# Ruyi-Zha/endosurf

Hardware: AMD Instinct MI355X
Metric: training rays/sec (1024 rays x 64 samples) (higher is better)
Workload: dtype f32

## Files before the change

endosurf_amd/csrc/chain_common.h:

```cpp
#pragma once
#include <hip/hip_runtime.h>

#include <type_traits>

#include "../../include/endosurf_hip.h"
#include "arch.h"

namespace es {

typedef float f32x16 __attribute__((ext_vector_type(16)));

__device__ __forceinline__ float relu1(float z) {
    float r;
    asm("v_max_f32_e32 %0, 0, %1" : "=v"(r) : "v"(z));
    return r;
}

constexpr int TM = 64;
constexpr int NTHREADS = 256;
constexpr int MAIN_FLOATS = HID * TM;
constexpr int AUX56_FLOATS = 56 * TM;
constexpr int LEAN_LDS_BYTES = (MAIN_FLOATS + AUX56_FLOATS + 256) * 4;

__device__ __forceinline__ int swz(int k, int r) { return k * TM + (r ^ ((k & 15) << 2)); }

template <int RTC, int NTC>
__device__ __forceinline__ void acc_zero(f32x16 (&acc)[RTC][NTC]) {
#pragma unroll
    for (int i = 0; i < RTC; ++i)
#pragma unroll
        for (int j = 0; j < NTC; ++j)
#pragma unroll
            for (int r = 0; r < 16; ++r) acc[i][j][r] = 0.f;
}

__device__ __forceinline__ float f4c(const float4& v, int j) { return j == 0 ? v.x : (j == 1 ? v.y : (j == 2 ? v.z : v.w)); }

template <int KG, int RTC, int NTC, int PF = 2>
__device__ __forceinline__ void gemm_seg(f32x16 (&acc)[RTC][NTC], const float* At, const float4* __restrict__ W,
                                         int rt0, int nt0, int lane) {
    static_assert(PF == 2 || PF == 4, "prefetch groups: even-group parity of the swizzle table");
    constexpr bool GUARD = (KG % (2 * PF)) != 0;
    const int lo = lane & 31, hi = lane >> 5;
    float4 b0[PF][NTC], b1[PF][NTC];
    const float4* wl = W + lane;
    int aoff[RTC][8];
#pragma unroll
    for (int ri = 0; ri < RTC; ++ri)
#pragma unroll
        for (int c = 0; c < 8; ++c) aoff[ri][c] = ((((rt0 + ri) * 32 + lo) ^ (hi << 2)) ^ (8 * c)) + 64 * hi;

    auto loadB = [&](float4(&b)[PF][NTC], int g0) {
#pragma unroll
        for (int gi = 0; gi < PF; ++gi)
#pragma unroll
            for (int ni = 0; ni < NTC; ++ni)
                if (!GUARD || g0 + gi < KG) b[gi][ni] = wl[(size_t)((nt0 + ni) * KG + g0 + gi) * 64];
    };
    auto comp = [&](const float4(&b)[PF][NTC], int g0) {
        const float* Ag = At + 512 * g0;
#pragma unroll
        for (int gi = 0; gi < PF; ++gi) {
            if (!GUARD || g0 + gi < KG) {
#pragma unroll
                for (int j = 0; j < 4; ++j) {
                    float a[RTC];
#pragma unroll
                    for (int ri = 0; ri < RTC; ++ri) a[ri] = Ag[aoff[ri][4 * (gi & 1) + j] + 512 * gi + 128 * j];
#pragma unroll
                    for (int ri = 0; ri < RTC; ++ri)
#pragma unroll
                        for (int ni = 0; ni < NTC; ++ni)
                            acc[ri][ni] = __builtin_amdgcn_mfma_f32_32x32x2f32(a[ri], f4c(b[gi][ni], j), acc[ri][ni], 0, 0, 0);
                }
            }
        }
    };

    loadB(b0, 0);
    if constexpr (KG > 2 * PF) {
#pragma unroll 1
        for (int g0 = 0; g0 < KG; g0 += 2 * PF) {
            if (!GUARD || g0 + PF < KG) loadB(b1, g0 + PF);
            comp(b0, g0);
            if (g0 + 2 * PF < KG) loadB(b0, g0 + 2 * PF);
            if (!GUARD || g0 + PF < KG) comp(b1, g0 + PF);
        }
    } else {
        if (PF < KG) loadB(b1, PF);
        comp(b0, 0);
        if (PF < KG) comp(b1, PF);
    }
}

template <int RTC, int NTC, class F>
__device__ __forceinline__ void for_quads(f32x16 (&acc)[RTC][NTC], int rt0, int nt0, int lane, F&& f) {
    const int lo = lane & 31, hi = lane >> 5;
#pragma unroll
    for (int ri = 0; ri < RTC; ++ri)
#pragma unroll
        for (int ni = 0; ni < NTC; ++ni)
#pragma unroll
            for (int q = 0; q < 4; ++q) {
                float v[4] = {acc[ri][ni][4 * q + 0], acc[ri][ni][4 * q + 1], acc[ri][ni][4 * q + 2], acc[ri][ni][4 * q + 3]};
                f((rt0 + ri) * 32 + 8 * q + 4 * hi, (nt0 + ni) * 32 + lo, v);
            }
}

template <int RTC, int NTC, class F>
__device__ __forceinline__ void for_quads_noacc(int rt0, int nt0, int lane, F&& f) {
    const int lo = lane & 31, hi = lane >> 5;
#pragma unroll
    for (int ri = 0; ri < RTC; ++ri)
#pragma unroll
        for (int ni = 0; ni < NTC; ++ni)
#pragma unroll
            for (int q = 0; q < 4; ++q) f((rt0 + ri) * 32 + 8 * q + 4 * hi, (nt0 + ni) * 32 + lo);
}

template <int RTC, int NTC, class F>
__device__ __forceinline__ void for_quads_qi(f32x16 (&acc)[RTC][NTC], int rt0, int nt0, int lane, F&& f) {
    const int lo = lane & 31, hi = lane >> 5;
#pragma unroll
    for (int ri = 0; ri < RTC; ++ri)
#pragma unroll
        for (int ni = 0; ni < NTC; ++ni)
#pragma unroll
            for (int q = 0; q < 4; ++q) {
                float v[4] = {acc[ri][ni][4 * q + 0], acc[ri][ni][4 * q + 1], acc[ri][ni][4 * q + 2], acc[ri][ni][4 * q + 3]};
                f((rt0 + ri) * 32 + 8 * q + 4 * hi, (nt0 + ni) * 32 + lo, v, (ri * NTC + ni) * 4 + q);
            }
}
template <int NI, class F>
__device__ __forceinline__ void for_quads_half(f32x16 (&acc)[2][2], int nt0, int lane, F&& f) {
    const int lo = lane & 31, hi = lane >> 5;
#pragma unroll
    for (int ri = 0; ri < 2; ++ri)
#pragma unroll
        for (int q = 0; q < 4; ++q) {
            float v[4] = {acc[ri][NI][4 * q + 0], acc[ri][NI][4 * q + 1], acc[ri][NI][4 * q + 2], acc[ri][NI][4 * q + 3]};
            f(ri * 32 + 8 * q + 4 * hi, (nt0 + NI) * 32 + lo, v, ri * 4 + q);
        }
}

typedef float f32x2v __attribute__((ext_vector_type(2)));
__device__ __forceinline__ void add_bias4(float (&v)[4], float b) {
    const f32x2v bb = {b, b};
    f32x2v lo = {v[0], v[1]}, hi = {v[2], v[3]};
    lo += bb; hi += bb;
    v[0] = lo[0]; v[1] = lo[1]; v[2] = hi[0]; v[3] = hi[1];
}
__device__ __forceinline__ float keep_if_bit(float v, unsigned w, int k) {
    const int m = __builtin_amdgcn_sbfe((int)w, k, 1);
    return __uint_as_float(__float_as_uint(v) & (unsigned)m);
}
template <int RTC> struct QuadOff { int o[RTC * 4]; };
template <int RTC>
__device__ __forceinline__ QuadOff<RTC> quad_offsets(int rt0, int nt0, int lane) {
    QuadOff<RTC> qo;
    const int lo = lane & 31, hi = lane >> 5;
#pragma unroll
    for (int ri = 0; ri < RTC; ++ri)
#pragma unroll
        for (int q = 0; q < 4; ++q) {
            int v = swz(nt0 * 32 + lo, (rt0 + ri) * 32 + 8 * q + 4 * hi);
            asm volatile("" : "+v"(v));
            qo.o[ri * 4 + q] = v;
        }
    return qo;
}
template <int RTC, int NTC, class F>
__device__ __forceinline__ void for_quads_off(f32x16 (&acc)[RTC][NTC], const QuadOff<RTC>& qo, int rt0, int nt0, int lane, F&& f) {
    const int lo = lane & 31, hi = lane >> 5;
#pragma unroll
    for (int ri = 0; ri < RTC; ++ri)
#pragma unroll
        for (int ni = 0; ni < NTC; ++ni)
#pragma unroll
            for (int q = 0; q < 4; ++q) {
                float v[4] = {acc[ri][ni][4 * q + 0], acc[ri][ni][4 * q + 1], acc[ri][ni][4 * q + 2], acc[ri][ni][4 * q + 3]};
                f((rt0 + ri) * 32 + 8 * q + 4 * hi, (nt0 + ni) * 32 + lo, v, qo.o[ri * 4 + q] + 2048 * ni, ni);
            }
}
__device__ __forceinline__ void lds_store_quad_at(float* At, int off, const float (&v)[4]) {
    *reinterpret_cast<float4*>(At + off) = make_float4(v[0], v[1], v[2], v[3]);
}
__device__ __forceinline__ void lds_store_quad(float* At, int col, int row, const float (&v)[4]) {
    *reinterpret_cast<float4*>(&At[swz(col, row)]) = make_float4(v[0], v[1], v[2], v[3]);
}
__device__ __forceinline__ void lds_load_quad(const float* At, int col, int row, float (&v)[4]) {
    const float4 t = *reinterpret_cast<const float4*>(&At[swz(col, row)]);
    v[0] = t.x; v[1] = t.y; v[2] = t.z; v[3] = t.w;
}
__device__ __forceinline__ void lds_add_quad(float* At, int col, int row, const float (&v)[4]) {
    float4* p = reinterpret_cast<float4*>(&At[swz(col, row)]);
    float4 t = *p;
    t.x += v[0]; t.y += v[1]; t.z += v[2]; t.w += v[3];
    *p = t;
}
__device__ __forceinline__ void g_store_quad(float* __restrict__ base, size_t grow0, int ld, int row, int col, const float (&v)[4]) {
    float* p = base + (grow0 + row) * (size_t)ld + col;
    __builtin_nontemporal_store(v[0], p); __builtin_nontemporal_store(v[1], p + ld);
    __builtin_nontemporal_store(v[2], p + 2 * ld); __builtin_nontemporal_store(v[3], p + 3 * ld);
}
__device__ __forceinline__ void g_load_quad(const float* __restrict__ base, size_t grow0, int ld, int row, int col, float (&v)[4]) {
    const float* p = base + (grow0 + row) * (size_t)ld + col;
    v[0] = __builtin_nontemporal_load(p); v[1] = __builtin_nontemporal_load(p + ld);
    v[2] = __builtin_nontemporal_load(p + 2 * ld); v[3] = __builtin_nontemporal_load(p + 3 * ld);
}

typedef float v4f_frag __attribute__((ext_vector_type(4)));
__device__ __forceinline__ size_t frag_off(size_t grow0, int row, int col) {
    const int ri = row >> 5, q = (row >> 3) & 3, hi = (row >> 2) & 1;
    const int w = col >> 6, ni = (col >> 5) & 1, lo = col & 31;
    return grow0 * 256 + (size_t)(((w * 16 + (ri * 2 + ni) * 4 + q) * 64 + hi * 32 + lo) * 4);
}
__device__ __forceinline__ void g_store_quad_f(float* __restrict__ base, size_t grow0, int row, int col, const float (&v)[4]) {
    const v4f_frag t = {v[0], v[1], v[2], v[3]};
    __builtin_nontemporal_store(t, reinterpret_cast<v4f_frag*>(base + frag_off(grow0, row, col)));
}
__device__ __forceinline__ void g_load_quad_f(const float* __restrict__ base, size_t grow0, int row, int col, float (&v)[4]) {
    const v4f_frag t = __builtin_nontemporal_load(reinterpret_cast<const v4f_frag*>(base + frag_off(grow0, row, col)));
    v[0] = t[0]; v[1] = t[1]; v[2] = t[2]; v[3] = t[3];
}
template <int RTC, int NTC>
__device__ __forceinline__ void prefetch_quads_f(float (&buf)[RTC * NTC * 4][4], const float* __restrict__ base, size_t grow0, int rt0, int nt0,
                                                 int lane) {
    const int lo = lane & 31, hi = lane >> 5;
#pragma unroll
    for (int ri = 0; ri < RTC; ++ri)
#pragma unroll
        for (int ni = 0; ni < NTC; ++ni)
#pragma unroll
            for (int q = 0; q < 4; ++q)
                g_load_quad_f(base, grow0, (rt0 + ri) * 32 + 8 * q + 4 * hi, (nt0 + ni) * 32 + lo, buf[(ri * NTC + ni) * 4 + q]);
}
template <int NI>
__device__ __forceinline__ void prefetch_half_f(float (&buf)[8][4], const float* __restrict__ base, size_t grow0, int nt0, int lane) {
    const int lo = lane & 31, hi = lane >> 5;
#pragma unroll
    for (int ri = 0; ri < 2; ++ri)
#pragma unroll
        for (int q = 0; q < 4; ++q) g_load_quad_f(base, grow0, ri * 32 + 8 * q + 4 * hi, (nt0 + NI) * 32 + lo, buf[ri * 4 + q]);
}

template <int NC>
__device__ __forceinline__ void load_tile(float* At, const float* __restrict__ src, size_t grow0, int ld, int tid) {
    const int r = tid >> 2, c4 = tid & 3;
    const float* p = src + (grow0 + r) * (size_t)ld;
#pragma unroll 4
    for (int jj = 0; jj < NC / 16; ++jj) {
        const int c = 4 * (c4 + 4 * jj);
        const float4 v = *reinterpret_cast<const float4*>(p + c);
        At[swz(c + 0, r)] = v.x; At[swz(c + 1, r)] = v.y; At[swz(c + 2, r)] = v.z; At[swz(c + 3, r)] = v.w;
    }
}
__device__ __forceinline__ void load_tile_256(float* At, const float* __restrict__ src, size_t grow0, int ld, int tid) {
    load_tile<256>(At, src, grow0, ld, tid);
}

struct MaskWords { unsigned w[2][2]; };
__device__ __forceinline__ MaskWords load_mask_words(const unsigned* __restrict__ Ml, int tile64, int wave, int lane) {
    MaskWords m;
    const unsigned* p = Ml + (size_t)(2 * tile64) * 256 + wave * 64 + (lane & 31);
    m.w[0][0] = p[0]; m.w[0][1] = p[32]; m.w[1][0] = p[256]; m.w[1][1] = p[256 + 32];
    return m;
}
__device__ __forceinline__ float mask_keep(float v, const MaskWords& m, int qi, int i, int hi) {
    const int ri_c = qi >> 3, ni = (qi >> 2) & 1, q_c = qi & 3;
    const int pq = ((q_c >> 1) * 2 + ni) * 4 + 2 * (q_c & 1) + hi;
    return keep_if_bit(v, m.w[ri_c][i >> 1], 2 * pq + (i & 1));
}
__device__ __forceinline__ bool mask_bit(const MaskWords& m, int qi, int i, int hi) {
    const int ri_c = qi >> 3, ni = (qi >> 2) & 1, q_c = qi & 3;
    const int pq = ((q_c >> 1) * 2 + ni) * 4 + 2 * (q_c & 1) + hi;
    return (m.w[ri_c][i >> 1] >> (2 * pq + (i & 1))) & 1u;
}

__device__ __forceinline__ float softplus100(float z) {
    const float e = __builtin_amdgcn_exp2f(-144.26950408889634f * fabsf(z));
    return fmaf(0.006931471805599453f, __builtin_amdgcn_logf(1.f + e), relu1(z));
}
__device__ __forceinline__ float softplus100_grad_from_s(float s) {
    const float x = 100.f * s;
    return x < 0.02f ? x * (1.f - x * (0.5f - x * (1.f / 6.f))) : 1.f - __expf(-x);
}

typedef float f32x2p __attribute__((ext_vector_type(2)));
__device__ __forceinline__ f32x2p softplus100_grad_from_s2(f32x2p s) {
    const f32x2p x = s * 100.f;
    const f32x2p t = x * -1.4426950408889634f;
    f32x2p e;
    e[0] = __builtin_amdgcn_exp2f(t[0]); e[1] = __builtin_amdgcn_exp2f(t[1]);
    const f32x2p big = 1.f - e;
    const f32x2p ser = x * (1.f - x * (0.5f - x * (1.f / 6.f)));
    f32x2p r;
    r[0] = x[0] < 0.02f ? ser[0] : big[0];
    r[1] = x[1] < 0.02f ? ser[1] : big[1];
    return r;
}
__device__ __forceinline__ void softplus100_grad_from_s4(const float (&s)[4], float (&d)[4]) {
    const f32x2p a = softplus100_grad_from_s2(f32x2p{s[0], s[1]}), b = softplus100_grad_from_s2(f32x2p{s[2], s[3]});
    d[0] = a[0]; d[1] = a[1]; d[2] = b[0]; d[3] = b[1];
}

__device__ __forceinline__ int enc_index(int D, int i, int fn, int c) { return D + (2 * i + fn) * D + c; }

template <int NOUT>
__device__ __forceinline__ void smalln_partial(const float* At, const float* __restrict__ Wrows, int ldw, float* scr, int tid) {
    const int row = tid & 63;
    const int part = __builtin_amdgcn_readfirstlane(tid >> 6);
    float s[NOUT];
#pragma unroll
    for (int i = 0; i < NOUT; ++i) s[i] = 0.f;
    const int k0 = part * 64;
#pragma unroll 8
    for (int kk = 0; kk < 64; ++kk) {
        const float a = At[swz(k0 + kk, row)];
#pragma unroll
        for (int i = 0; i < NOUT; ++i) s[i] = fmaf(Wrows[i * ldw + k0 + kk], a, s[i]);
    }
#pragma unroll
    for (int i = 0; i < NOUT; ++i) scr[(part * NOUT + i) * 64 + row] = s[i];
}
template <int NOUT>
__device__ __forceinline__ float smalln_reduce(const float* scr, int i, int row) {
    return (scr[(0 * NOUT + i) * 64 + row] + scr[(1 * NOUT + i) * 64 + row]) + (scr[(2 * NOUT + i) * 64 + row] + scr[(3 * NOUT + i) * 64 + row]);
}

struct PointSrc : ::es_points {};
static_assert(sizeof(PointSrc) == sizeof(es_points) && std::is_standard_layout<PointSrc>::value, "es::PointSrc is es_points");
__device__ __forceinline__ void load_point(const PointSrc& s, int i_in, float (&x)[3], float& t, float (&d)[3]) {
    int i = i_in;
    if (i >= s.M) { x[0] = x[1] = x[2] = 0.f; t = 0.f; d[0] = d[1] = 0.f; d[2] = 1.f; return; }
    if (s.mode == 0 || (s.mode == 2 && i >= s.M_split)) {
        if (s.mode == 2) i -= s.M_split;
        x[0] = s.x[3 * (size_t)i]; x[1] = s.x[3 * (size_t)i + 1]; x[2] = s.x[3 * (size_t)i + 2];
        t = s.t[s.t_scalar ? 0 : i];
        if (s.dirs) { d[0] = s.dirs[3 * (size_t)i]; d[1] = s.dirs[3 * (size_t)i + 1]; d[2] = s.dirs[3 * (size_t)i + 2]; }
        else { d[0] = d[1] = 0.f; d[2] = 1.f; }
    } else {
        const int ray = i / s.n_per_ray, smp = i - ray * s.n_per_ray;
        const float* r = s.rays + 9 * (size_t)ray;
        const float zz = s.z[(size_t)ray * s.ldz + smp];
        const float inv = r[5] + 1e-6f;
        d[0] = r[3]; d[1] = r[4]; d[2] = r[5];
        x[0] = r[0] + (r[3] / inv) * zz; x[1] = r[1] + (r[4] / inv) * zz; x[2] = r[2] + (r[5] / inv) * zz;
        t = r[8];
    }
}

}
```

endosurf_amd/csrc/point_bwd_bodies.h:

```cpp
#pragma once
#include <type_traits>

#include "chain_common.h"
#include "encode.h"
#include "tabs.h"
#include "workspace.h"

namespace es {

struct BwdArgs {
    PointSrc src;
    Tabs tb;
    const float4* packed;
    const float* weff;
    float* ws;
    WsLayout L;
    int flags;
    int M_color;
    const float* d_sdf;
    const float* d_go;
    const float* d_rgb;
};
__device__ __forceinline__ float* wsb(const BwdArgs& a, int buf) { return a.ws + a.L.off[buf]; }

// ... 271 lines not shown
        acc_zero(acc);
        const int seg = l <= 4 ? SF0 + l : SF0 + l + 1;
        gemm_seg<32, 2, 2>(acc, mainT, a.packed + a.tb.segoff[seg], 0, 2 * wave, lane);
        if (l == 4) gemm_seg<5, 2, 2>(acc, aux, a.packed + a.tb.segoff[SF4A], 0, 2 * wave, lane);
        __syncthreads();
        epi_t(acc, l);
        __syncthreads();
    }
    auto epi_b = [&](f32x16(&acc)[2][2], int l) {
        auto half = [&](auto NI) {
            float S[8][4], Z2[8][4];
            prefetch_half_f<decltype(NI)::value>(S, SACT + (size_t)(l - 1) * Mp * 256, grow0, 2 * wave, lane);
            prefetch_half_f<decltype(NI)::value>(Z2, ZB + (size_t)(l - 1) * Mp * 256, grow0, 2 * wave, lane);
            for_quads_half<decltype(NI)::value>(acc, 2 * wave, lane, [&](int row, int col, float(&v)[4], int b8) {
                float dphi[4];
                softplus100_grad_from_s4(S[b8], dphi);
#pragma unroll
                for (int h = 0; h < 2; ++h) {
                    const f32x2p d = {dphi[2 * h], dphi[2 * h + 1]}, t = {v[2 * h], v[2 * h + 1]}, z = {Z2[b8][2 * h], Z2[b8][2 * h + 1]};
                    const f32x2p o = d * t + z;
                    v[2 * h] = o[0]; v[2 * h + 1] = o[1];
                }
                lds_store_quad(mainT, col, row, v);
                g_store_quad_f(ZB + (size_t)(l - 1) * Mp * 256, grow0, row, col, v);
            });
        };
        half(std::integral_constant<int, 0>{});
        half(std::integral_constant<int, 1>{});
    };
    {
        f32x16 acc[2][2];
        acc_zero(acc);
        if (color) {
            load_tile_256(mainT, wsb(a, WS_FEATBAR), grow0, 256, tid);
            __syncthreads();
            gemm_seg<32, 2, 2>(acc, mainT, a.packed + a.tb.segoff[SR8F], 0, 2 * wave, lane);
            __syncthreads();
        }
        const float* w8 = a.weff + a.tb.woff[NET_S * LAYERS + 8];
        for_quads(acc, 0, 2 * wave, lane, [&](int row, int col, float(&v)[4]) {
            const float w = w8[col];
#pragma unroll
            for (int i = 0; i < 4; ++i) v[i] += sb[row + i] * w;
            float s[4], z2[4];
            g_load_quad_f(SACT + (size_t)7 * Mp * 256, grow0, row, col, s);
            g_load_quad_f(ZB + (size_t)7 * Mp * 256, grow0, row, col, z2);
#pragma unroll
            for (int i = 0; i < 4; ++i) v[i] = softplus100_grad_from_s(s[i]) * v[i] + z2[i];
            lds_store_quad(mainT, col, row, v);
            g_store_quad_f(ZB + (size_t)7 * Mp * 256, grow0, row, col, v);
        });
    }
    __syncthreads();
#pragma unroll 1
    for (int l = 7; l >= 1; --l) {
        f32x16 acc[2][2];
        acc_zero(acc);
        const int seg = l <= 4 ? SR0 + l : SR0 + l + 1;
        gemm_seg<32, 2, 2>(acc, mainT, a.packed + a.tb.segoff[seg], 0, 2 * wave, lane);
        f32x16 accA[1][1];
        if (l == 4) {
            acc_zero(accA);
            gemm_seg<32, 1, 1>(accA, mainT, a.packed + a.tb.segoff[SR4A], wave >> 1, wave & 1, lane);
        }
        __syncthreads();
        epi_b(acc, l);
        if (l == 4)
            for_quads(accA, wave >> 1, wave & 1, lane, [&](int row, int col, float(&v)[4]) { if (col < 40) lds_store_quad(aux, col, row, v); });
        __syncthreads();
    }
    {
        f32x16 accA[1][1];
        acc_zero(accA);
        gemm_seg<32, 1, 1>(accA, mainT, a.packed + a.tb.segoff[SR0], wave >> 1, wave & 1, lane);
        for_quads(accA, wave >> 1, wave & 1, lane, [&](int row, int col, float(&v)[4]) { if (col < 40) lds_add_quad(aux, col, row, v); });
    }
    __syncthreads();
    if (tid < 192) {
        const int j = tid >> 6, row = tid & 63;
        const float x = px[j * 64 + row];
        float g = enc3_adjoint<6>(aux, 0, j, row, x);
        const float* AE = wsb(a, WS_S_ADJEPS) + (grow0 + row) * 64;
        float h = 0.f;
#pragma unroll
        for (int i = 0; i < 6; ++i) {
            const float f = (float)(1 << i);
            float s, co;
            sincosf(x * f, &s, &co);
            h -= f * f * (AE[enc_index(3, i, 0, j)] * s + AE[enc_index(3, i, 1, j)] * co);
        }
        tx[j * 64 + row] = g + h * gb[j * 64 + row];
    }
    __syncthreads();
    if (tid < 64) {
        const size_t gp = grow0 + tid;
        float* xb = wsb(a, WS_XCBAR) + gp * 3;
#pragma unroll
        for (int j = 0; j < 3; ++j) xb[j] = tx[j * 64 + tid] + (color ? wsb(a, WS_XCBAR_C)[gp * 3 + j] : 0.f);
    }
}

__device__ __forceinline__ void deform_tan_tile(const BwdArgs& a, const int tile) {
    extern __shared__ __attribute__((aligned(16))) float lds[];
    float* mainT = lds;
    float* aux = lds + MAIN_FLOATS;
    float* scr = aux + AUX56_FLOATS;
    float* ub = scr;
    float* px = mainT;
    float* red = aux;
    const int tid = threadIdx.x, lane = tid & 63;
    const int wave = __builtin_amdgcn_readfirstlane(tid >> 6);
    const int row0 = tile * TM;
    const size_t grow0 = (size_t)row0;
    const size_t Mp = (size_t)a.L.Mp;
    const unsigned* MK = reinterpret_cast<const unsigned*>(wsb(a, WS_D_MASK));
    const size_t nt32 = Mp / 32;
    const int hi = lane >> 5;
    float* T = wsb(a, WS_D_T);

    if (tid < 64) {
        const bool valid = row0 + tid < a.src.M;
        float x[3], t, d[3];
        load_point(a.src, row0 + tid, x, t, d);
        px[tid] = x[0]; px[64 + tid] = x[1]; px[128 + tid] = x[2];
#pragma unroll
        for (int i = 0; i < 3; ++i) ub[i * 64 + tid] = valid ? a.d_go[3 * (size_t)(row0 + tid) + i] : 0.f;
    }
    zero_rows(aux, 0, 56, tid);
    __syncthreads();
    {
        const int row = tid & 63, part = tid >> 6;
        for (int item = part; item < 18; item += 4) {
            const int c = item % 3, i = item / 3;
            const float f = (float)(1 << i);
            float s, co;
            sincosf(px[c * 64 + row] * f, &s, &co);
            const float g = ub[c * 64 + row];
            aux[swz(enc_index(3, i, 0, c), row)] = f * co * g;
            aux[swz(enc_index(3, i, 1, c), row)] = -f * s * g;
        }
        if (part == 3) {
#pragma unroll
            for (int c = 0; c < 3; ++c) aux[swz(c, row)] = ub[c * 64 + row];
        }
    }
    __syncthreads();
    {
        float* T0 = wsb(a, WS_D_T0);
        const int r = tid >> 2, c4 = tid & 3;
        for (int k = c4; k < 56; k += 4) T0[(grow0 + r) * 64 + k] = aux[swz(k, r)];
    }
    const QuadOff<2> qo = quad_offsets<2>(0, 2 * wave, lane);
    auto epi_impl = [&](f32x16(&acc)[2][2], int l, const MaskWords& mk, auto SKIP) {
        float* Tl = T + (size_t)l * Mp * 256;
        for_quads_off(acc, qo, 0, 2 * wave, lane, [&](int row, int col, float(&v)[4], int off, int ni) {
            const int qi = (((row >> 5) * 2 + ni) << 2) + ((row >> 3) & 3);
            if (decltype(SKIP)::value && col >= 204) {
                lds_load_quad(aux, col - 204, row, v);
            } else {
#pragma unroll
                for (int i = 0; i < 4; ++i) v[i] = mask_keep(v[i], mk, qi, i, hi);
            }
            lds_store_quad_at(mainT, off, v);
            g_store_quad(Tl, grow0, 256, row, col, v);
        });
    };
    auto epi = [&](f32x16(&acc)[2][2], int l, const MaskWords& mk) {
        if (l == 3 && wave == 3) epi_impl(acc, l, mk, std::true_type{});
        else epi_impl(acc, l, mk, std::false_type{});
    };
    {
        const MaskWords mk = load_mask_words(MK, tile, wave, lane);
        f32x16 acc[2][2];
        acc_zero(acc);
        gemm_seg<7, 2, 2>(acc, aux, a.packed + a.tb.segoff[DF0], 0, 2 * wave, lane);
        epi(acc, 0, mk);
    }
    __syncthreads();
#pragma unroll 1
    for (int l = 1; l <= 7; ++l) {
        const MaskWords mk = load_mask_words(MK + (size_t)l * nt32 * 256, tile, wave, lane);
        f32x16 acc[2][2];
        acc_zero(acc);
        gemm_seg<32, 2, 2>(acc, mainT, a.packed + a.tb.segoff[DF0 + l], 0, 2 * wave, lane);
        __syncthreads();
        epi(acc, l, mk);
        __syncthreads();
    }
    smalln_partial<3>(mainT, a.weff + a.tb.woff[NET_D * LAYERS + 8], 256, red, tid);
    __syncthreads();
    if (tid < 192) {
        const int i = tid >> 6, row = tid & 63;
        wsb(a, WS_JU)[(grow0 + row) * 3 + i] = smalln_reduce<3>(red, i, row) + ub[i * 64 + row];
    }
}

constexpr int DBWD_LDS_BYTES = (MAIN_FLOATS + 192) * 4;
template <bool HALF = false>
__device__ __forceinline__ void deform_bwd_tile(const BwdArgs& a, const int tile) {
    constexpr int PTS = HALF ? 16 : 32, RTC = HALF ? 1 : 2;
    extern __shared__ __attribute__((aligned(16))) float lds[];
    float* mainT = lds;
    float* a8 = lds + MAIN_FLOATS;
    const int tid = threadIdx.x, lane = tid & 63;
    const int wave = __builtin_amdgcn_readfirstlane(tid >> 6);
    const int pt0 = tile * PTS;
    const size_t grow0 = (size_t)pt0 * 2;
    const size_t rows2 = (size_t)a.L.Mp * 2;
    const bool color = a.flags & PF_COLOR;
    auto mask_word = [&](const unsigned* MK, size_t nt32, int l) -> unsigned {
        if constexpr (HALF) return MK[((size_t)l * nt32 + (tile >> 1)) * 256 + tid] >> (16 * (tile & 1));
        else return MK[((size_t)l * nt32 + tile) * 256 + tid];
    };

    if (tid < 2 * PTS) {
        const int p = tid >> 1, c = tid & 1;
        const size_t gp = (size_t)(pt0 + p);
        const bool has_v = color && pt0 + p < a.M_color;
        float* A8 = wsb(a, WS_D_A8) + (grow0 + tid) * 4;
#pragma unroll
        for (int i = 0; i < 3; ++i) {
            const float v = c == 0 ? wsb(a, WS_XCBAR)[gp * 3 + i] : (has_v ? wsb(a, WS_VBAR_C)[gp * 3 + i] : 0.f);
            a8[i * 64 + tid] = v; A8[i] = v;
        }
        A8[3] = 0.f;
    }
    __syncthreads();
    const unsigned* MK = reinterpret_cast<const unsigned*>(wsb(a, WS_D_MASK));
    const size_t nt32 = (size_t)a.L.Mp / 32;
    float* DA = wsb(a, WS_D_A);
    {
        const float* W8 = a.weff + a.tb.woff[NET_D * LAYERS + 8];
        const unsigned bits = mask_word(MK, nt32, 7);
        for_quads_noacc<RTC, 2>(0, 2 * wave, lane, [&](int row, int col) {
            const float w0 = W8[col], w1 = W8[256 + col], w2 = W8[512 + col];
            const int qi = ((row >> 5) * 2 + ((col >> 5) & 1)) * 4 + ((row & 31) >> 3);
            const bool m0 = (bits >> (2 * qi)) & 1u, m2 = (bits >> (2 * qi + 1)) & 1u;
            float v[4];
#pragma unroll
            for (int i = 0; i < 4; ++i) v[i] = (i < 2 ? m0 : m2) ? a8[row + i] * w0 + a8[64 + row + i] * w1 + a8[128 + row + i] * w2 : 0.f;
            lds_store_quad(mainT, col, row, v);
            g_store_quad(DA + (size_t)7 * rows2 * 256, grow0, 256, row, col, v);
        });
    }
    __syncthreads();
#pragma unroll 1
    for (int l = 7; l >= 1; --l) {
        const unsigned bits = mask_word(MK, nt32, l - 1);
        f32x16 acc[RTC][2];
        acc_zero(acc);
        if (l == 3) gemm_seg<26, RTC, 2>(acc, mainT, a.packed + a.tb.segoff[DR3], 0, 2 * wave, lane);
        else gemm_seg<32, RTC, 2>(acc, mainT, a.packed + a.tb.segoff[DR0 + l], 0, 2 * wave, lane);
        __syncthreads();
        float* Al = DA + (size_t)(l - 1) * rows2 * 256;
        for_quads_qi(acc, 0, 2 * wave, lane, [&](int row, int col, float(&v)[4], int qi) {
            const bool dead = l == 4 && col >= 204;
            const bool m0 = !dead && ((bits >> (2 * qi)) & 1u), m2 = !dead && ((bits >> (2 * qi + 1)) & 1u);
            v[0] = m0 ? v[0] : 0.f; v[1] = m0 ? v[1] : 0.f; v[2] = m2 ? v[2] : 0.f; v[3] = m2 ? v[3] : 0.f;
            lds_store_quad(mainT, col, row, v);
            g_store_quad(Al, grow0, 256, row, col, v);
        });
        __syncthreads();
    }
}

}
```

endosurf_amd/csrc/point_fwd_bodies.h:

```cpp
#pragma once
#include <type_traits>
#include "chain_common.h"
#include "encode.h"
#include "tabs.h"
#include "workspace.h"

namespace es {

struct FwdArgs {
    PointSrc src;
    Tabs tb;
    const float4* packed;
    const float* weff;
    float* ws;
    WsLayout L;
    int flags;
    int M_color;
};

__device__ __forceinline__ float* wsb(const FwdArgs& a, int buf) { return a.ws + a.L.off[buf]; }

template <bool HALF = false>
__device__ __forceinline__ void deform_fwd_tile(const FwdArgs& a, const int tile) {
    constexpr int PTS = HALF ? 16 : 32, RTC = HALF ? 1 : 2;
    extern __shared__ __attribute__((aligned(16))) float lds[];
    float* mainT = lds;
    float* aux = lds + MAIN_FLOATS;
    float* scr = aux + AUX56_FLOATS;
    float* px = scr;
    float* pd = scr + 96;
    float* pt = scr + 192;
    float* red = aux;
    const int tid = threadIdx.x, lane = tid & 63;
    const int wave = __builtin_amdgcn_readfirstlane(tid >> 6);
    const int pt0 = tile * PTS;
    const size_t grow0 = (size_t)pt0 * 2;
    const bool save = a.flags & PF_SAVE;
    const size_t rows2 = (size_t)a.L.Mp * 2;

    if (tid < PTS) {
        float x[3], t, d[3];
        load_point(a.src, pt0 + tid, x, t, d);
        px[tid] = x[0]; px[32 + tid] = x[1]; px[64 + tid] = x[2]; pt[tid] = t;
        pd[tid] = d[0]; pd[32 + tid] = d[1]; pd[64 + tid] = d[2];
    }
    zero_rows(aux, 0, 56, tid);
    __syncthreads();
    {
        const int p = tid & 31;
        for (int item = tid >> 5; item < 25 && p < PTS; item += 8) {
            if (item < 18) {
                const int c = item % 3, i = item / 3;
                const float f = (float)(1 << i);
                float s, co;
                sincosf(px[c * 32 + p] * f, &s, &co);
                const float dc = pd[c * 32 + p];
                aux[swz(enc_index(3, i, 0, c), 2 * p)] = s;
                aux[swz(enc_index(3, i, 1, c), 2 * p)] = co;
                aux[swz(enc_index(3, i, 0, c), 2 * p + 1)] = f * co * dc;
                aux[swz(enc_index(3, i, 1, c), 2 * p + 1)] = -f * s * dc;
            } else if (item < 24) {
                const int i = item - 18;
                float s, co;
                sincosf(pt[p] * (float)(1 << i), &s, &co);
                aux[swz(39 + enc_index(1, i, 0, 0), 2 * p)] = s;
                aux[swz(39 + enc_index(1, i, 1, 0), 2 * p)] = co;
            } else {
#pragma unroll
                for (int c = 0; c < 3; ++c) { aux[swz(c, 2 * p)] = px[c * 32 + p]; aux[swz(c, 2 * p + 1)] = pd[c * 32 + p]; }
                aux[swz(39, 2 * p)] = pt[p];
            }
        }
    }
    __syncthreads();
    if (save) {
        float* U0 = wsb(a, WS_D_U0);
        const int r = tid >> 2, c4 = tid & 3;
        if (r < 2 * PTS)
            for (int k = c4; k < 56; k += 4) U0[(grow0 + r) * 64 + k] = aux[swz(k, r)];
    }

    float* U = wsb(a, WS_D_U);
    unsigned* MK = reinterpret_cast<unsigned*>(wsb(a, WS_D_MASK));
    const size_t nt32 = (size_t)a.L.Mp / 32;
    const QuadOff<RTC> qo = quad_offsets<RTC>(0, 2 * wave, lane);
    auto bias2 = [&](float(&b)[2], int l) {
        const float* bias = a.weff + a.tb.boff[NET_D * LAYERS + l] + 64 * wave + (lane & 31);
        b[0] = bias[0]; b[1] = bias[32];
    };
    auto epi_impl = [&](f32x16(&acc)[RTC][2], int l, const float(&bc)[2], auto SKIP, auto SAVE) {
        float* Ul = U + (size_t)l * rows2 * 256;
        unsigned bits = 0;
        for_quads_off(acc, qo, 0, 2 * wave, lane, [&](int row, int col, float(&v)[4], int off, int ni) {
            const int qi = (((row >> 5) * 2 + ni) << 2) + ((row >> 3) & 3);
            if (decltype(SKIP)::value && col >= 204) {
                lds_load_quad(aux, col - 204, row, v);
            } else {
                const float a0 = v[0] + bc[ni], a2 = v[2] + bc[ni];
                const bool m0 = a0 > 0.f, m2 = a2 > 0.f;
                v[0] = m0 ? a0 : 0.f; v[1] = m0 ? v[1] : 0.f; v[2] = m2 ? a2 : 0.f; v[3] = m2 ? v[3] : 0.f;
                bits |= (m0 ? 1u : 0u) << (2 * qi) | (m2 ? 1u : 0u) << (2 * qi + 1);
            }
            lds_store_quad_at(mainT, off, v);
            if (decltype(SAVE)::value) g_store_quad(Ul, grow0, 256, row, col, v);
        });
        if constexpr (HALF) reinterpret_cast<unsigned short*>(MK)[(((size_t)l * nt32 + (tile >> 1)) * 256 + tid) * 2 + (tile & 1)] = (unsigned short)bits;
        else MK[((size_t)l * nt32 + tile) * 256 + tid] = bits;
    };
    auto epi = [&](f32x16(&acc)[RTC][2], int l, const float(&bc)[2], auto SKIP) {
        if (save) epi_impl(acc, l, bc, SKIP, std::true_type{});
        else epi_impl(acc, l, bc, SKIP, std::false_type{});
    };
    float bc[2], bn[2];
    bias2(bn, 0);
    {
        f32x16 acc[RTC][2];
        acc_zero(acc);
        bc[0] = bn[0]; bc[1] = bn[1];
        bias2(bn, 1);
        gemm_seg<7, RTC, 2>(acc, aux, a.packed + a.tb.segoff[DF0], 0, 2 * wave, lane);
        epi(acc, 0, bc, std::false_type{});
    }
    __syncthreads();
#pragma unroll 1
    for (int l = 1; l <= 7; ++l) {
        f32x16 acc[RTC][2];
        acc_zero(acc);
        bc[0] = bn[0]; bc[1] = bn[1];
        if (l < 7) bias2(bn, l + 1);
        gemm_seg<32, RTC, 2>(acc, mainT, a.packed + a.tb.segoff[DF0 + l], 0, 2 * wave, lane);
        __syncthreads();
        if (l == 3 && wave == 3) epi(acc, l, bc, std::true_type{});
        else epi(acc, l, bc, std::false_type{});
        __syncthreads();
    }
    smalln_partial<3>(mainT, a.weff + a.tb.woff[NET_D * LAYERS + 8], 256, red, tid);
    __syncthreads();
    if (tid < 192) {
        const int i = tid >> 6, row = tid & 63, p = row >> 1, c = row & 1;
        const float val = smalln_reduce<3>(red, i, row);
        const size_t gp = (size_t)(pt0 + p);
        if (p >= PTS) {
        } else if (c == 0) wsb(a, WS_XC)[gp * 3 + i] = px[i * 32 + p] + val + a.weff[a.tb.boff[NET_D * LAYERS + 8] + i];
        else wsb(a, WS_V)[gp * 3 + i] = val + pd[i * 32 + p];
    }
}

template <bool HALF = false>
__device__ __forceinline__ void deform_vjp_tile(const FwdArgs& a, const int tile_in) {
    constexpr int RTC = HALF ? 1 : 2;
    const int tile = HALF ? (tile_in >> 1) : tile_in;
    const int RT0 = HALF ? (tile_in & 1) : 0;
    extern __shared__ __attribute__((aligned(16))) float lds[];
    float* mainT = lds;
    float* aux = lds + MAIN_FLOATS;
    float* scr = aux + AUX56_FLOATS;
    float* g8 = scr;
    const int tid = threadIdx.x, lane = tid & 63;
    const int wave = __builtin_amdgcn_readfirstlane(tid >> 6);
    const int row0 = tile * TM;
    const size_t grow0 = (size_t)row0;
    const bool save = a.flags & PF_SAVE;
    const size_t Mp = (size_t)a.L.Mp;
    const unsigned* MK = reinterpret_cast<const unsigned*>(wsb(a, WS_D_MASK));
    const size_t nt32 = Mp / 32;
    const int hi = lane >> 5;
    float* R = wsb(a, WS_D_R);

    const QuadOff<RTC> qo = quad_offsets<RTC>(RT0, 2 * wave, lane);
    if (tid < 64) {
        const float* gc = wsb(a, WS_GC) + (grow0 + tid) * 3;
        g8[tid] = gc[0]; g8[64 + tid] = gc[1]; g8[128 + tid] = gc[2];
    }
    zero_rows(aux, 0, 56, tid);
    __syncthreads();
    {
        const float* W8 = a.weff + a.tb.woff[NET_D * LAYERS + 8];
        const MaskWords mk = load_mask_words(MK + (size_t)7 * nt32 * 256, tile, wave, lane);
        for_quads_noacc<RTC, 2>(RT0, 2 * wave, lane, [&](int row, int col) {
            const float w0 = W8[col], w1 = W8[256 + col], w2 = W8[512 + col];
            const int qi = ((row >> 5) * 2 + ((col >> 5) & 1)) * 4 + ((row & 31) >> 3);
            float v[4];
#pragma unroll
            for (int i = 0; i < 4; ++i) v[i] = mask_bit(mk, qi, i, hi) ? g8[row + i] * w0 + g8[64 + row + i] * w1 + g8[128 + row + i] * w2 : 0.f;
            lds_store_quad(mainT, col, row, v);
            if (save) g_store_quad(R + (size_t)7 * Mp * 256, grow0, 256, row, col, v);
        });
    }
    __syncthreads();
#pragma unroll 1
    for (int l = 7; l >= 1; --l) {
        const MaskWords mk = load_mask_words(MK + (size_t)(l - 1) * nt32 * 256, tile, wave, lane);
        f32x16 acc[RTC][2];
        acc_zero(acc);
        if (l == 3) gemm_seg<26, RTC, 2>(acc, mainT, a.packed + a.tb.segoff[DR3], RT0, 2 * wave, lane);
        else gemm_seg<32, RTC, 2>(acc, mainT, a.packed + a.tb.segoff[DR0 + l], RT0, 2 * wave, lane);
        __syncthreads();
        float* Rl = R + (size_t)(l - 1) * Mp * 256;
        auto epi = [&](auto SKIP, auto SAVE) {
            for_quads_off(acc, qo, RT0, 2 * wave, lane, [&](int row, int col, float(&v)[4], int off, int ni) {
                const int qi = (((row >> 5) * 2 + ni) << 2) + ((row >> 3) & 3);
                if (decltype(SKIP)::value && col >= 204) {
                    lds_store_quad(aux, col - 204, row, v);
#pragma unroll
                    for (int i = 0; i < 4; ++i) v[i] = 0.f;
                } else {
#pragma unroll
                    for (int i = 0; i < 4; ++i) v[i] = mask_keep(v[i], mk, qi, i, hi);
                }
                lds_store_quad_at(mainT, off, v);
                if (decltype(SAVE)::value) g_store_quad(Rl, grow0, 256, row, col, v);
            });
        };
        if (l == 4 && wave == 3) { if (save) epi(std::true_type{}, std::true_type{}); else epi(std::true_type{}, std::false_type{}); }
        else { if (save) epi(std::false_type{}, std::true_type{}); else epi(std::false_type{}, std::false_type{}); }
        __syncthreads();
    }
    {
        if (!HALF || (wave >> 1) == 0) {
            const int art = HALF ? RT0 : (wave >> 1);
            f32x16 accA[1][1];
            acc_zero(accA);
            gemm_seg<32, 1, 1>(accA, mainT, a.packed + a.tb.segoff[DR0], art, wave & 1, lane);
            for_quads(accA, art, wave & 1, lane, [&](int row, int col, float(&v)[4]) { if (col < 52) lds_add_quad(aux, col, row, v); });
        }
    }
    __syncthreads();
    if (tid < 192) {
        const int j = tid >> 6, row = tid & 63;
        float x[3], t, d[3];
        load_point(a.src, row0 + row, x, t, d);
        float g = g8[j * 64 + row] + aux[swz(j, row)];
        float c2 = 0.f;
#pragma unroll
        for (int i = 0; i < 6; ++i) {
            const float f = (float)(1 << i);
            float s, co;
            sincosf(x[j] * f, &s, &co);
            const float as = aux[swz(enc_index(3, i, 0, j), row)], ac = aux[swz(enc_index(3, i, 1, j), row)];
            g += f * (as * co - ac * s);
            c2 += (f * f) * (as * s + ac * co);
        }
        if (!HALF || (row >> 5) == RT0) {
            wsb(a, WS_GO)[(grow0 + row) * 3 + j] = g;
            wsb(a, WS_CURV)[(grow0 + row) * 3 + j] = c2;
        }
    } else {
        const int row = tid & 63;
        float x[3], t, d[3];
        load_point(a.src, row0 + row, x, t, d);
        float g = aux[swz(39, row)];
#pragma unroll
        for (int i = 0; i < 6; ++i) {
            const float f = (float)(1 << i);
            float s, co;
            sincosf(t * f, &s, &co);
            g += f * (aux[swz(39 + enc_index(1, i, 0, 0), row)] * co - aux[swz(39 + enc_index(1, i, 1, 0), row)] * s);
        }
        if (!HALF || (row >> 5) == RT0) wsb(a, WS_TBAR)[grow0 + row] = g;
    }
}

template <bool HALF = false>
__device__ __forceinline__ void sdf_fwd_tile(const FwdArgs& a, const int tile_in) {
    constexpr int RTC = HALF ? 1 : 2;
    const int tile = HALF ? (tile_in >> 1) : tile_in;
    const int RT0 = HALF ? (tile_in & 1) : 0;
    auto own = [&](int row) { return !HALF || (row >> 5) == RT0; };
    extern __shared__ __attribute__((aligned(16))) float lds[];
    float* mainT = lds;
    float* aux = lds + MAIN_FLOATS;
    float* scr = aux + AUX56_FLOATS;
    float* px = scr;
    float* red = aux;
    float* gcv = mainT;
    const int tid = threadIdx.x, lane = tid & 63;
    const int wave = __builtin_amdgcn_readfirstlane(tid >> 6);
    const int row0 = tile * TM;
    const size_t grow0 = (size_t)row0;
    const bool save = a.flags & PF_SAVE, deform = a.flags & PF_DEFORM, color = (a.flags & PF_COLOR) && row0 < a.M_color;
    const size_t Mp = (size_t)a.L.Mp;

    if (tid < 64) {
        if (deform) {
            const float* xc = wsb(a, WS_XC) + (grow0 + tid) * 3;
            px[tid] = xc[0]; px[64 + tid] = xc[1]; px[128 + tid] = xc[2];
        } else {
            float x[3], t, d[3];
            load_point(a.src, row0 + tid, x, t, d);
            px[tid] = x[0]; px[64 + tid] = x[1]; px[128 + tid] = x[2];
            if (own(tid)) {
                float* xc = wsb(a, WS_XC) + (grow0 + tid) * 3;
                xc[0] = x[0]; xc[1] = x[1]; xc[2] = x[2];
            }
        }
    }
    __syncthreads();
    encode3<6>(aux, 0, px, tid);
    zero_rows(aux, 39, 40, tid);
    __syncthreads();
    if (save) {
        float* S0 = wsb(a, WS_S_S0);
        const int r = tid >> 2, c4 = tid & 3;
        if (own(r))
            for (int k = c4; k < 40; k += 4) S0[(grow0 + r) * 64 + k] = aux[swz(k, r)];
    }
    float* SACT = wsb(a, WS_S_ACT);
    const QuadOff<RTC> qo = quad_offsets<RTC>(RT0, 2 * wave, lane);
    auto bias2 = [&](float(&b)[2], int l) {
        const float* bias = a.weff + a.tb.boff[NET_S * LAYERS + l] + 64 * wave + (lane & 31);
        b[0] = bias[0]; b[1] = bias[32];
    };
    auto epi = [&](f32x16(&acc)[RTC][2], int l, const float(&bc)[2]) {
        float* Sl = SACT + (size_t)l * Mp * 256;
        for_quads_off(acc, qo, RT0, 2 * wave, lane, [&](int row, int col, float(&v)[4], int off, int ni) {
            add_bias4(v, bc[ni]);
#pragma unroll
            for (int i = 0; i < 4; ++i) v[i] = softplus100(v[i]);
            lds_store_quad_at(mainT, off, v);
            g_store_quad_f(Sl, grow0, row, col, v);
        });
    };
    float bc[2], bn[2];
    bias2(bn, 0);
    {
        f32x16 acc[RTC][2];
        acc_zero(acc);
        bc[0] = bn[0]; bc[1] = bn[1];
        bias2(bn, 1);
        gemm_seg<5, RTC, 2>(acc, aux, a.packed + a.tb.segoff[SF0], RT0, 2 * wave, lane);
        epi(acc, 0, bc);
    }
    __syncthreads();
#pragma unroll 1
    for (int l = 1; l <= 7; ++l) {
        f32x16 acc[RTC][2];
        acc_zero(acc);
        bc[0] = bn[0]; bc[1] = bn[1];
        if (l < 7) bias2(bn, l + 1);
        const int seg = l <= 4 ? SF0 + l : SF0 + l + 1;
        gemm_seg<32, RTC, 2>(acc, mainT, a.packed + a.tb.segoff[seg], RT0, 2 * wave, lane);
        if (l == 4) gemm_seg<5, RTC, 2>(acc, aux, a.packed + a.tb.segoff[SF4A], RT0, 2 * wave, lane);
        __syncthreads();
        epi(acc, l, bc);
        __syncthreads();
    }
    if (color) {
        f32x16 acc[RTC][2];
        acc_zero(acc);
        gemm_seg<32, RTC, 2>(acc, mainT, a.packed + a.tb.segoff[SF8F], RT0, 2 * wave, lane);
        const float* bias = a.weff + a.tb.boff[NET_S * LAYERS + 8] + 1;
        float* feat = wsb(a, WS_FEAT);
        for_quads(acc, RT0, 2 * wave, lane, [&](int row, int col, float(&v)[4]) {
            const float b = bias[col];
#pragma unroll
            for (int i = 0; i < 4; ++i) v[i] += b;
            g_store_quad(feat, grow0, 256, row, col, v);
        });
    }
    smalln_partial<1>(mainT, a.weff + a.tb.woff[NET_S * LAYERS + 8], 256, red, tid);
    __syncthreads();
    if (tid < 64 && own(tid)) wsb(a, WS_SDF)[grow0 + tid] = smalln_reduce<1>(red, 0, tid) + a.weff[a.tb.boff[NET_S * LAYERS + 8]];

    float* RHO = wsb(a, WS_S_RHO);
    {
        const float* w8 = a.weff + a.tb.woff[NET_S * LAYERS + 8];
        const float w8c[2] = {w8[64 * wave + (lane & 31)], w8[64 * wave + 32 + (lane & 31)]};
        auto rho7 = [&](auto SAVE) {
            f32x16 dummy[RTC][2];
            for_quads_off(dummy, qo, RT0, 2 * wave, lane, [&](int row, int col, float(&v)[4], int off, int ni) {
                const float4 t = *reinterpret_cast<const float4*>(mainT + off);
                const float sv[4] = {t.x, t.y, t.z, t.w};
                softplus100_grad_from_s4(sv, v);
#pragma unroll
                for (int i = 0; i < 4; ++i) v[i] *= w8c[ni];
                lds_store_quad_at(mainT, off, v);
                if (decltype(SAVE)::value) g_store_quad_f(RHO + (size_t)7 * Mp * 256, grow0, row, col, v);
            });
// ... 204 lines not shown
```

Baseline: 73100.

## Stream saved activations to global memory inside the next layer's GEMM

Global stores of per-layer activations used to run in each epilogue. They are removed there, and a StreamOut hook inside gemm_seg now reads the previous layer's tile back from LDS and stores it slot by slot, interleaved with the MFMA groups of the following layer. The last layer's tile is flushed after the loop. The aim is to hide global write latency behind matrix compute and shorten the epilogues, at the cost of extra LDS reads, more register pressure and more complex scheduling through sched_barrier.

```diff
diff --git a/endosurf_amd/csrc/chain_common.h b/endosurf_amd/csrc/chain_common.h
--- a/endosurf_amd/csrc/chain_common.h
+++ b/endosurf_amd/csrc/chain_common.h
@@ -36,9 +36,13 @@
 
 __device__ __forceinline__ float f4c(const float4& v, int j) { return j == 0 ? v.x : (j == 1 ? v.y : (j == 2 ? v.z : v.w)); }
 
-template <int KG, int RTC, int NTC, int PF = 2>
+struct NoHook {
+    __device__ __forceinline__ void pre() const {}
+    template <int SMAX> __device__ __forceinline__ void slot(int) const {}
+};
+template <int KG, int RTC, int NTC, int PF = 2, class Hook = NoHook>
 __device__ __forceinline__ void gemm_seg(f32x16 (&acc)[RTC][NTC], const float* At, const float4* __restrict__ W,
-                                         int rt0, int nt0, int lane) {
+                                         int rt0, int nt0, int lane, Hook&& hook = Hook{}) {
     static_assert(PF == 2 || PF == 4, "prefetch groups: even-group parity of the swizzle table");
     constexpr bool GUARD = (KG % (2 * PF)) != 0;
     const int lo = lane & 31, hi = lane >> 5;
@@ -78,18 +82,36 @@
     };
 
     loadB(b0, 0);
-    if constexpr (KG > 2 * PF) {
+    hook.pre();
+    if constexpr (KG > 2 * PF && !std::is_same<typename std::decay<Hook>::type, NoHook>::value) {
+        constexpr int GT = (KG - 1) / (2 * PF) * (2 * PF);
+#pragma unroll 1
+        for (int g0 = 0; g0 < GT; g0 += 2 * PF) {
+            loadB(b1, g0 + PF);
+            hook.template slot<GT / PF - 2>(g0 / PF);
+            comp(b0, g0);
+            loadB(b0, g0 + 2 * PF);
+            hook.template slot<GT / PF - 1>(g0 / PF + 1);
+            comp(b1, g0 + PF);
+        }
+        if constexpr (GT + PF < KG) loadB(b1, GT + PF);
+        hook.template slot<GT / PF>(GT / PF);
+        comp(b0, GT);
+        if constexpr (GT + PF < KG) { hook.template slot<GT / PF + 1>(GT / PF + 1); comp(b1, GT + PF); }
+    } else if constexpr (KG > 2 * PF) {
 #pragma unroll 1
         for (int g0 = 0; g0 < KG; g0 += 2 * PF) {
             if (!GUARD || g0 + PF < KG) loadB(b1, g0 + PF);
+            hook.template slot<(KG - 1) / PF>(g0 / PF);
             comp(b0, g0);
             if (g0 + 2 * PF < KG) loadB(b0, g0 + 2 * PF);
-            if (!GUARD || g0 + PF < KG) comp(b1, g0 + PF);
+            if (!GUARD || g0 + PF < KG) { hook.template slot<(KG - 1) / PF>(g0 / PF + 1); comp(b1, g0 + PF); }
         }
     } else {
         if (PF < KG) loadB(b1, PF);
+        hook.template slot<0>(0);
         comp(b0, 0);
-        if (PF < KG) comp(b1, PF);
+        if (PF < KG) { hook.template slot<1>(1); comp(b1, PF); }
     }
 }
 
@@ -208,6 +230,59 @@
     v[0] = __builtin_nontemporal_load(p); v[1] = __builtin_nontemporal_load(p + ld);
     v[2] = __builtin_nontemporal_load(p + 2 * ld); v[3] = __builtin_nontemporal_load(p + 3 * ld);
 }
+
+template <int RTC>
+struct StreamOut {
+    static constexpr int NQ = RTC * 8;
+    const float* At;
+    float* ubase;
+    int o0;
+    unsigned loff;
+    float4 pend;
+    __device__ __forceinline__ void init(const float* tile, int rt0, int nt0, int lane) {
+        const int lo = lane & 31, hi = lane >> 5;
+        At = tile;
+        o0 = swz(nt0 * 32 + lo, rt0 * 32 + 4 * hi);
+        loff = (unsigned)((rt0 * 32 + 4 * hi) * 256 + nt0 * 32 + lo) * 4u;
+    }
+    __device__ __forceinline__ void init(const float* tile, const QuadOff<RTC>& qo, int rt0, int nt0, int lane) {
+        init(tile, rt0, nt0, lane);
+        o0 = qo.o[0];
+    }
+    static __device__ __forceinline__ int lds_x(int s) { return ((s & 3) << 3) | ((s >> 3) << 5) | (((s >> 2) & 1) << 11); }
+    static __device__ __forceinline__ int hbm_x(int s) { return ((s & 3) << 11) | ((s >> 3) << 13) | (((s >> 2) & 1) << 5); }
+    __device__ __forceinline__ void read(int s) { pend = *reinterpret_cast<const float4*>(At + (o0 ^ lds_x(s))); }
+    __device__ __forceinline__ void store(int s) const {
+        float* p = reinterpret_cast<float*>(reinterpret_cast<char*>(ubase) + (loff + 4u * (unsigned)hbm_x(s)));
+        __builtin_nontemporal_store(pend.x, p); __builtin_nontemporal_store(pend.y, p + 256);
+        __builtin_nontemporal_store(pend.z, p + 512); __builtin_nontemporal_store(pend.w, p + 768);
+    }
+    __device__ __forceinline__ void begin(float* rows0) { ubase = rows0; read(0); }
+    __device__ __forceinline__ void step(int q) {
+        __builtin_amdgcn_sched_barrier(0);
+        store(q); read(q + 1);
+        __builtin_amdgcn_sched_barrier(0);
+    }
+    __device__ __forceinline__ void pre() { step(0); }
+    template <int SMAX>
+    __device__ __forceinline__ void slot(int s) {
+        if constexpr (SMAX + 1 < NQ) step(s + 1);
+        else if (s + 1 < NQ) step(s + 1);
+    }
+    __device__ __forceinline__ void flush(float* rows0) {
+        begin(rows0);
+#pragma unroll
+        for (int q = 0; q < NQ; ++q) { store(q); if (q + 1 < NQ) read(q + 1); }
+    }
+    template <int SLOTS>
+    __device__ __forceinline__ void finish() {
+        if constexpr (SLOTS + 1 < NQ) {
+            store(SLOTS + 1);
+#pragma unroll
+            for (int q = SLOTS + 2; q < NQ; ++q) { read(q); store(q); }
+        }
+    }
+};
 
 typedef float v4f_frag __attribute__((ext_vector_type(4)));
 __device__ __forceinline__ size_t frag_off(size_t grow0, int row, int col) {
diff --git a/endosurf_amd/csrc/point_bwd_bodies.h b/endosurf_amd/csrc/point_bwd_bodies.h
--- a/endosurf_amd/csrc/point_bwd_bodies.h
+++ b/endosurf_amd/csrc/point_bwd_bodies.h
@@ -447,7 +447,6 @@
     }
     const QuadOff<2> qo = quad_offsets<2>(0, 2 * wave, lane);
     auto epi_impl = [&](f32x16(&acc)[2][2], int l, const MaskWords& mk, auto SKIP) {
-        float* Tl = T + (size_t)l * Mp * 256;
         for_quads_off(acc, qo, 0, 2 * wave, lane, [&](int row, int col, float(&v)[4], int off, int ni) {
             const int qi = (((row >> 5) * 2 + ni) << 2) + ((row >> 3) & 3);
             if (decltype(SKIP)::value && col >= 204) {
@@ -457,13 +456,14 @@
                 for (int i = 0; i < 4; ++i) v[i] = mask_keep(v[i], mk, qi, i, hi);
             }
             lds_store_quad_at(mainT, off, v);
-            g_store_quad(Tl, grow0, 256, row, col, v);
         });
     };
     auto epi = [&](f32x16(&acc)[2][2], int l, const MaskWords& mk) {
         if (l == 3 && wave == 3) epi_impl(acc, l, mk, std::true_type{});
         else epi_impl(acc, l, mk, std::false_type{});
     };
+    StreamOut<2> so;
+    so.init(mainT, qo, 0, 2 * wave, lane);
     {
         const MaskWords mk = load_mask_words(MK, tile, wave, lane);
         f32x16 acc[2][2];
@@ -477,11 +477,13 @@
         const MaskWords mk = load_mask_words(MK + (size_t)l * nt32 * 256, tile, wave, lane);
         f32x16 acc[2][2];
         acc_zero(acc);
-        gemm_seg<32, 2, 2>(acc, mainT, a.packed + a.tb.segoff[DF0 + l], 0, 2 * wave, lane);
+        so.begin(T + ((size_t)(l - 1) * Mp + grow0) * 256);
+        gemm_seg<32, 2, 2>(acc, mainT, a.packed + a.tb.segoff[DF0 + l], 0, 2 * wave, lane, so);
         __syncthreads();
         epi(acc, l, mk);
         __syncthreads();
     }
+    so.flush(T + ((size_t)7 * Mp + grow0) * 256);
     smalln_partial<3>(mainT, a.weff + a.tb.woff[NET_D * LAYERS + 8], 256, red, tid);
     __syncthreads();
     if (tid < 192) {
@@ -535,28 +537,31 @@
 #pragma unroll
             for (int i = 0; i < 4; ++i) v[i] = (i < 2 ? m0 : m2) ? a8[row + i] * w0 + a8[64 + row + i] * w1 + a8[128 + row + i] * w2 : 0.f;
             lds_store_quad(mainT, col, row, v);
-            g_store_quad(DA + (size_t)7 * rows2 * 256, grow0, 256, row, col, v);
-        });
-    }
-    __syncthreads();
+        });
+    }
+    __syncthreads();
+    StreamOut<RTC> so;
+    so.init(mainT, 0, 2 * wave, lane);
 #pragma unroll 1
     for (int l = 7; l >= 1; --l) {
         const unsigned bits = mask_word(MK, nt32, l - 1);
         f32x16 acc[RTC][2];
         acc_zero(acc);
-        if (l == 3) gemm_seg<26, RTC, 2>(acc, mainT, a.packed + a.tb.segoff[DR3], 0, 2 * wave, lane);
-        else gemm_seg<32, RTC, 2>(acc, mainT, a.packed + a.tb.segoff[DR0 + l], 0, 2 * wave, lane);
-        __syncthreads();
-        float* Al = DA + (size_t)(l - 1) * rows2 * 256;
+        so.begin(DA + ((size_t)l * rows2 + grow0) * 256);
+        if (l == 3) {
+            gemm_seg<26, RTC, 2>(acc, mainT, a.packed + a.tb.segoff[DR3], 0, 2 * wave, lane, so);
+            so.template finish<13>();
+        } else gemm_seg<32, RTC, 2>(acc, mainT, a.packed + a.tb.segoff[DR0 + l], 0, 2 * wave, lane, so);
+        __syncthreads();
         for_quads_qi(acc, 0, 2 * wave, lane, [&](int row, int col, float(&v)[4], int qi) {
             const bool dead = l == 4 && col >= 204;
             const bool m0 = !dead && ((bits >> (2 * qi)) & 1u), m2 = !dead && ((bits >> (2 * qi + 1)) & 1u);
             v[0] = m0 ? v[0] : 0.f; v[1] = m0 ? v[1] : 0.f; v[2] = m2 ? v[2] : 0.f; v[3] = m2 ? v[3] : 0.f;
             lds_store_quad(mainT, col, row, v);
-            g_store_quad(Al, grow0, 256, row, col, v);
-        });
-        __syncthreads();
-    }
-}
-
-}
+        });
+        __syncthreads();
+    }
+    so.flush(DA + grow0 * 256);
+}
+
+}
diff --git a/endosurf_amd/csrc/point_fwd_bodies.h b/endosurf_amd/csrc/point_fwd_bodies.h
--- a/endosurf_amd/csrc/point_fwd_bodies.h
+++ b/endosurf_amd/csrc/point_fwd_bodies.h
@@ -88,8 +88,7 @@
         const float* bias = a.weff + a.tb.boff[NET_D * LAYERS + l] + 64 * wave + (lane & 31);
         b[0] = bias[0]; b[1] = bias[32];
     };
-    auto epi_impl = [&](f32x16(&acc)[RTC][2], int l, const float(&bc)[2], auto SKIP, auto SAVE) {
-        float* Ul = U + (size_t)l * rows2 * 256;
+    auto epi = [&](f32x16(&acc)[RTC][2], int l, const float(&bc)[2], auto SKIP) {
         unsigned bits = 0;
         for_quads_off(acc, qo, 0, 2 * wave, lane, [&](int row, int col, float(&v)[4], int off, int ni) {
             const int qi = (((row >> 5) * 2 + ni) << 2) + ((row >> 3) & 3);
@@ -102,15 +101,12 @@
                 bits |= (m0 ? 1u : 0u) << (2 * qi) | (m2 ? 1u : 0u) << (2 * qi + 1);
             }
             lds_store_quad_at(mainT, off, v);
-            if (decltype(SAVE)::value) g_store_quad(Ul, grow0, 256, row, col, v);
         });
         if constexpr (HALF) reinterpret_cast<unsigned short*>(MK)[(((size_t)l * nt32 + (tile >> 1)) * 256 + tid) * 2 + (tile & 1)] = (unsigned short)bits;
         else MK[((size_t)l * nt32 + tile) * 256 + tid] = bits;
     };
-    auto epi = [&](f32x16(&acc)[RTC][2], int l, const float(&bc)[2], auto SKIP) {
-        if (save) epi_impl(acc, l, bc, SKIP, std::true_type{});
-        else epi_impl(acc, l, bc, SKIP, std::false_type{});
-    };
+    StreamOut<RTC> so;
+    so.init(mainT, qo, 0, 2 * wave, lane);
     float bc[2], bn[2];
     bias2(bn, 0);
     {
@@ -128,12 +124,16 @@
         acc_zero(acc);
         bc[0] = bn[0]; bc[1] = bn[1];
         if (l < 7) bias2(bn, l + 1);
-        gemm_seg<32, RTC, 2>(acc, mainT, a.packed + a.tb.segoff[DF0 + l], 0, 2 * wave, lane);
+        if (save) {
+            so.begin(U + ((size_t)(l - 1) * rows2 + grow0) * 256);
+            gemm_seg<32, RTC, 2>(acc, mainT, a.packed + a.tb.segoff[DF0 + l], 0, 2 * wave, lane, so);
+        } else gemm_seg<32, RTC, 2>(acc, mainT, a.packed + a.tb.segoff[DF0 + l], 0, 2 * wave, lane);
         __syncthreads();
         if (l == 3 && wave == 3) epi(acc, l, bc, std::true_type{});
         else epi(acc, l, bc, std::false_type{});
         __syncthreads();
     }
+    if (save) so.flush(U + ((size_t)7 * rows2 + grow0) * 256);
     smalln_partial<3>(mainT, a.weff + a.tb.woff[NET_D * LAYERS + 8], 256, red, tid);
     __syncthreads();
     if (tid < 192) {
@@ -184,20 +184,28 @@
 #pragma unroll
             for (int i = 0; i < 4; ++i) v[i] = mask_bit(mk, qi, i, hi) ? g8[row + i] * w0 + g8[64 + row + i] * w1 + g8[128 + row + i] * w2 : 0.f;
             lds_store_quad(mainT, col, row, v);
-            if (save) g_store_quad(R + (size_t)7 * Mp * 256, grow0, 256, row, col, v);
         });
     }
     __syncthreads();
+    StreamOut<RTC> so;
+    so.init(mainT, qo, RT0, 2 * wave, lane);
 #pragma unroll 1
     for (int l = 7; l >= 1; --l) {
         const MaskWords mk = load_mask_words(MK + (size_t)(l - 1) * nt32 * 256, tile, wave, lane);
         f32x16 acc[RTC][2];
         acc_zero(acc);
-        if (l == 3) gemm_seg<26, RTC, 2>(acc, mainT, a.packed + a.tb.segoff[DR3], RT0, 2 * wave, lane);
-        else gemm_seg<32, RTC, 2>(acc, mainT, a.packed + a.tb.segoff[DR0 + l], RT0, 2 * wave, lane);
-        __syncthreads();
-        float* Rl = R + (size_t)(l - 1) * Mp * 256;
-        auto epi = [&](auto SKIP, auto SAVE) {
+        if (save) {
+            so.begin(R + ((size_t)l * Mp + grow0) * 256);
+            if (l == 3) {
+                gemm_seg<26, RTC, 2>(acc, mainT, a.packed + a.tb.segoff[DR3], RT0, 2 * wave, lane, so);
+                so.template finish<13>();
+            } else gemm_seg<32, RTC, 2>(acc, mainT, a.packed + a.tb.segoff[DR0 + l], RT0, 2 * wave, lane, so);
+        } else {
+            if (l == 3) gemm_seg<26, RTC, 2>(acc, mainT, a.packed + a.tb.segoff[DR3], RT0, 2 * wave, lane);
+            else gemm_seg<32, RTC, 2>(acc, mainT, a.packed + a.tb.segoff[DR0 + l], RT0, 2 * wave, lane);
+        }
+        __syncthreads();
+        auto epi = [&](auto SKIP) {
             for_quads_off(acc, qo, RT0, 2 * wave, lane, [&](int row, int col, float(&v)[4], int off, int ni) {
                 const int qi = (((row >> 5) * 2 + ni) << 2) + ((row >> 3) & 3);
                 if (decltype(SKIP)::value && col >= 204) {
@@ -209,11 +217,9 @@
                     for (int i = 0; i < 4; ++i) v[i] = mask_keep(v[i], mk, qi, i, hi);
                 }
                 lds_store_quad_at(mainT, off, v);
-                if (decltype(SAVE)::value) g_store_quad(Rl, grow0, 256, row, col, v);
             });
         };
-        if (l == 4 && wave == 3) { if (save) epi(std::true_type{}, std::true_type{}); else epi(std::true_type{}, std::false_type{}); }
-        else { if (save) epi(std::false_type{}, std::true_type{}); else epi(std::false_type{}, std::false_type{}); }
+        if (l == 4 && wave == 3) epi(std::true_type{}); else epi(std::false_type{});
         __syncthreads();
     }
     {
@@ -224,6 +230,7 @@
             gemm_seg<32, 1, 1>(accA, mainT, a.packed + a.tb.segoff[DR0], art, wave & 1, lane);
             for_quads(accA, art, wave & 1, lane, [&](int row, int col, float(&v)[4]) { if (col < 52) lds_add_quad(aux, col, row, v); });
         }
+        if (save) so.flush(R + grow0 * 256);
     }
     __syncthreads();
     if (tid < 192) {
```

Result: no change. 73700 (median of 6 runs) (+0.8%).
